# zadorlab/sella

Hardware: AMD Instinct MI355X
Metric: Davidson iterations/s (3N=3072 synthetic Hessian, jd0, gamma=0.1, maxiter=40; whole rayleigh_ritz call incl. device eigh of the preconditioner) (higher is better)
Workload: dtype f64; 1 GPU; 1024-atom-equivalent 3N=3072 fp64 Davidson (BASELINE configs[1]), one independent replica per GPU; n=3072, maxiter=40, method=jd0, problems=20, matrices=4

## Files before the change

### sella_amd/csrc/eigh.hip

```cpp
#include "internal.h"
#include "host_math.h"
#include "secular.h"

#include <algorithm>
#include <chrono>
#include <numeric>

namespace sella {
namespace {

constexpr int TRD_NBMAX = 64;
constexpr int TRD_PA = 1;
constexpr int WY_NB = 32;

__device__ __forceinline__ double wave_sum_e(double v) { return wave_sum64(v); }

__device__ __forceinline__ double block_sum_256(double v, double* red ) {
    v = wave_sum_e(v);
    __syncthreads();
    if ((threadIdx.x & 63) == 0) red[threadIdx.x >> 6] = v;
    __syncthreads();
    return red[0] + red[1] + red[2] + red[3];
}

struct TrdRowArgs {
    double* A; int ld, n;
    int j;
    int i;
    int do_row;
    double* Vp; double* Wp; int ldp;
    const double* u_prev; double* u_cur;
    const double* wraw;
    const double* partA_prev; int nblkA_prev;
    double* partA_cur;
    const double* partB; int nblkB;
    const double* colscal;
    const double* cdots;
    double* dvec;
};

template <int IPC>
__global__ __launch_bounds__(256) void trd_row_kernel(TrdRowArgs a) {
    __shared__ double red[4];
    SELLA_ARG(a.A); SELLA_ARG(a.ld); SELLA_ARG(a.n); SELLA_ARG(a.j); SELLA_ARG(a.i); SELLA_ARG(a.do_row); SELLA_ARG(a.Vp);
    SELLA_ARG(a.Wp); SELLA_ARG(a.ldp); SELLA_ARG(a.u_cur); SELLA_ARG(a.wraw); SELLA_ARG(a.partA_cur); SELLA_ARG(a.partB);
    SELLA_ARG(a.nblkB); SELLA_ARG(a.colscal); SELLA_ARG(a.cdots); SELLA_ARG(a.dvec);
    const int tid = threadIdx.x;
    const int j = a.j, i = a.i, ldp = a.ldp;
    const int c = j + blockIdx.x * 256 + tid;
    const bool valid = c < a.n;
    const int cl = valid ? c : a.n - 1;
    const int ip = i - 1;
    double pv0[8];
    {
        const int last = (a.nblkB > 0) ? a.nblkB - 1 : 0;
#pragma unroll
        for (int k = 0; k < 8; ++k) {
            const int b = tid + 256 * k;
            pv0[k] = a.partB[b < a.nblkB ? b : last];
        }
    }
    auto sum_partials = [&]() -> double {
        double vw = 0.0;
        if (IPC > 0 || i > 0) {
#pragma unroll
// ... 22 lines not shown
    bool vw_done = false;
    if (IPC > 3) {
        __shared__ double uni[4 * 32];
        constexpr int NPC = IPC > 0 ? IPC : 1;
        double vcs[NPC], wcs[NPC];
#pragma unroll
        for (int p = 0; p < NPC; ++p) {
            vcs[p] = a.Vp[(size_t)p * ldp + cl];
            wcs[p] = a.Wp[(size_t)p * ldp + cl];
        }
        if (tid < 4 * NPC) {
            const int p = tid >> 2, k = tid & 3;
            uni[tid] = (k == 0) ? a.cdots[p] : (k == 1) ? a.cdots[TRD_NBMAX + p]
                     : (k == 2) ? a.Vp[(size_t)p * ldp + j] : a.Wp[(size_t)p * ldp + j];
        }
        vw = block_sum_256(sum_partials(), red);
        vw_done = true;
#pragma unroll
        for (int p = 0; p < NPC; ++p) {
            const double c1 = uni[4 * p], c2 = uni[4 * p + 1], vj = uni[4 * p + 2], wj_p = uni[4 * p + 3];
            s += vcs[p] * c1 + wcs[p] * c2;
            q += vcs[p] * wj_p + wcs[p] * vj;
            cc += c1 * c2;
            t += vj * c1 + wj_p * c2;
        }
    } else {
#pragma unroll
        for (int p = 0; p < np; ++p) {
            const double c1 = a.cdots[p], c2 = a.cdots[TRD_NBMAX + p];
            const double vj = a.Vp[(size_t)p * ldp + j], wj_p = a.Wp[(size_t)p * ldp + j];
            const double vc = a.Vp[(size_t)p * ldp + cl], wcp = a.Wp[(size_t)p * ldp + cl];
            s += vc * c1 + wcp * c2;
            q += vc * wj_p + wcp * vj;
            cc += c1 * c2;
            t += vj * c1 + wj_p * c2;
        }
    }
    double wc = 0.0, u = 0.0;
    if (i > 0) {
        if (!vw_done) vw = block_sum_256(sum_partials(), red);
        const double alpha2 = -0.5 * tau * tau * (vw - 2.0 * cc);
        const double wj = tau * (wrawj - t) + alpha2;
        wc = tau * (wrawc - s) + alpha2 * vprev;
        if (valid) a.Wp[(size_t)ip * ldp + c] = wc;
        u = arow - q - (vprev * wj + wc);
    } else {
        u = arow;
    }
    if (!a.do_row) return;
    if (valid) {
        a.u_cur[c] = u;
        if (c == j) a.dvec[j] = u;
    }
    double ss = (valid && c >= j + 2) ? u * u : 0.0;
    ss = block_sum_256(ss, red);
    if (tid == 0) a.partA_cur[(size_t)blockIdx.x * TRD_PA] = ss;
}

__device__ __forceinline__ double2 ldg2(const double* p) { return *reinterpret_cast<const double2*>(p); }

struct TrdGemvArgs {
    const double* A22;
    int ld, m, shift, o, n, j;
    int pad;
    const double* ubuf;
    const double* partA; int nblkA;
    double* wraw;
    double* partB;
    double* Vrow;
    double* Arow;
    double* taus; double* evec; double* colscal;
    const double* Wp; const double* Vp; int ldp, i;
    double* cdots;
};

template <int NCH>
__global__ __launch_bounds__(256) void trd_gemv_kernel(TrdGemvArgs a) {
    __shared__ double red[4][2];
    const int lane = threadIdx.x & 63, wave = threadIdx.x >> 6;
    const int row0 = blockIdx.x * 2 - a.pad;
    const int mtot = a.m + 2 * a.i;
    const int oc = a.o - a.shift;
    const double2* arow[2];
    double lead[2];
#pragma unroll
    for (int r = 0; r < 2; ++r) {
        int rr = row0 + r;
        if (rr < 0) rr = 0;
        if (rr > mtot - 1) rr = mtot - 1;
        const double* base;
        if (rr < a.m) base = a.A22 + (size_t)rr * a.ld;
        else if (rr < a.m + a.i) base = a.Wp + (size_t)(rr - a.m) * a.ldp + oc;
        else base = a.Vp + (size_t)(rr - a.m - a.i) * a.ldp + oc;
        arow[r] = reinterpret_cast<const double2*>(base);
        lead[r] = base[a.shift];
    }
    double ssl0 = a.partA[(size_t)(lane < a.nblkA ? lane : a.nblkA - 1) * TRD_PA];
    double ssl = 0.0;
    for (int b = lane + 64; b < a.nblkA; b += 64) ssl += a.partA[(size_t)b * TRD_PA];
    const double alpha = a.ubuf[a.o];
    double urow[2];
#pragma unroll
    for (int r = 0; r < 2; ++r) {
        const int rr = row0 + r;
        urow[r] = a.ubuf[(rr >= 0 && rr < a.m) ? a.o + rr : a.o];
    }
    double acc[2] = {0.0, 0.0};
    const int n2 = (a.m + a.shift + 1) >> 1;
    auto uval = [&](int cabs) -> double { return (cabs > a.o && cabs < a.n) ? a.ubuf[cabs] : 0.0; };
// ... 1914 lines not shown
                hipLaunchKernelGGL(zhat_batched_kernel, dim3((maxK + 3) / 4, nm), dim3(256), 0, c->stream, mdd, Dd, wd, taud,
                                   orgd, zhd);
                hipLaunchKernelGGL(build_u_batched_kernel, dim3(maxK, nm), dim3(256), 0, c->stream, mdd, Dd, zhd, taud, orgd,
                                   W.Ut, ld);
            }
            hipLaunchKernelGGL(gather_level_kernel, dim3((maxN + 255) / 256, n), dim3(256), 0, c->stream, mdd, mrowd, idxd, cur,
                               W.Zc, nxt, ld);
            HIPCHK(hipGetLastError());
            SCHK(launch_gemm_merge_batched(c, nm, gdescd, maxN, maxK, W.Ut, W.Zc, nxt, ld));
        }
        HIPCHK(hipGetLastError());
        HIPCHK(hipMemcpyAsync(lam, lamd, (size_t)n * sizeof(double), hipMemcpyDeviceToHost, c->stream));
        HIPCHK(hipMemcpyAsync(hi2, info, 2 * sizeof(int), hipMemcpyDeviceToHost, c->stream));
        std::swap(cur, nxt);
        if (dc_timing) {
            const auto tw3 = std::chrono::steady_clock::now();
            auto us = [](auto a, auto b) { return std::chrono::duration<double, std::micro>(b - a).count(); };
            fprintf(stderr, "dc level %d: wait %.1f us, values + plan + staging %.1f us, uploads + launches %.1f us\n", h, us(tw0, tw1),
                    us(tw1, tw2), us(tw2, tw3));
        }
        if (pipelined) {
            plans_prev.swap(plans);
            if (h < maxdepth) SCHK(queue_level_vectors(h + 1, cur));
        } else {
            SCHK(stream_wait(c));
            SCHK(take_level_values(plans, defl_all[h & 1]));
        }
    }
    if (pipelined && maxdepth >= 1) {
        SCHK(stream_wait(c));
        SCHK(take_level_values(plans_prev, defl_all[maxdepth & 1]));
    }
    order.resize(n);
    ascending_order(vals.data(), n, order.data(), order_all.data());
    for (int i = 0; i < n; ++i) wout[i] = vals[order[i]];
    std::copy(order.begin(), order.end(), hidx);
    HIPCHK(hipMemcpyAsync(idxd, hidx, (size_t)n * sizeof(int), hipMemcpyHostToDevice, c->stream));
    SCHK(launch_gather_rows(c, cur, ld, idxd, n, n, nxt, ld));
    SCHK(stream_wait(c));
    if (nxt != W.Za) std::swap(W.Za, W.Zb);
    return SELLA_OK;
}

static int tridiagonalise(EighWork& W, double* taus, double* dvec, double* evec) {
    sella_ctx* c = W.c;
    const int n = W.n, ld = W.ld;
    int nb = (int)c->opt.eigh_nb;
    if (nb > TRD_NBMAX) nb = TRD_NBMAX;
    const int nrefl = n - 2;
    double *Vp, *Wp, *part;
    SCHK(scratch_get(c, SCR_MISC0, (size_t)2 * TRD_NBMAX * ld * sizeof(double), &Vp));
    Wp = Vp + (size_t)nb * ld;
    HIPCHK(s_memset0(c, Vp, (size_t)2 * nb * ld * sizeof(double)));
    const int maxblkA = (n + 255) / 256 + 1, maxblkB = (n + 16 + 2 * TRD_NBMAX + 1) / 2 + 1;
    SCHK(scratch_get(c, SCR_MISC1, ((size_t)2 * maxblkA * TRD_PA + 2 * (size_t)maxblkB + 4 * TRD_NBMAX + 128) * sizeof(double), &part));
    double* partA[2] = {part, part + (size_t)maxblkA * TRD_PA};
    double* partB = part + 2 * (size_t)maxblkA * TRD_PA;
    double* ub[2] = {W.vec + (size_t)V_U0 * ld, W.vec + (size_t)V_U1 * ld};
    double* wraw = W.vec + (size_t)V_WRAW * ld;
    double* colscal = W.vec + (size_t)V_COL * ld;
    double* cdots = partB + maxblkB + 8;
    double* partB2[2] = {partB, cdots + 2 * TRD_NBMAX + 8};
    double* colscal2[2] = {colscal, partB2[1] + maxblkB + 8};
    double* wraw2[2] = {wraw, W.vec + (size_t)V_WRAW2 * ld};
    const int upd_max = (int)c->opt.eigh_upd_max;
    int cur = 0, nblkA_prev = 0, nblkB_prev = 0;
    const int symv_min = (int)c->opt.eigh_symv_min;
    const int symTR = c->opt.eigh_symv_tr == 128 ? 128 : 64;
    const int symNJ = (n + SYMV_TC - 1) / SYMV_TC, symNI = (n + symTR - 1) / symTR;
    const int ldP = (n + 255) / 256 * 256;
    double *Prow = nullptr, *Pcol = nullptr;
    if (symv_min > 0 && n - 1 >= symv_min) {
        SCHK(scratch_get(c, SCR_SYMV, (size_t)(symNJ + symNI) * ldP * sizeof(double), &Prow));
        Pcol = Prow + (size_t)symNJ * ldP;
    }
    const int tail_lds = (int)std::min<long>(c->opt.eigh_tail_lds, TRD_TAIL);
    bool lower_stale = false;
    const bool can_tri = c->opt.rank2k_stream;
    for (int j0 = 0; j0 < nrefl; j0 += nb) {
        const int kb = std::min(nb, nrefl - j0);
        if (upd_max > 0 && !lower_stale && n - j0 - 1 <= upd_max && !(tail_lds > 0 && n - j0 <= tail_lds) &&
            !(symv_min > 0 && n - j0 - 1 >= symv_min)) {
            const int jend = tail_lds > 0 ? std::min(nrefl, n - tail_lds) : nrefl;
            int fc = 0, nblk_last = 0;
            for (int j = j0; j < jend; ++j) {
                const int o = j + 1, m = n - o;
                TrdUpdArgs ua;
                ua.A = W.A; ua.ld = ld; ua.n = n; ua.j = j;
                ua.o = o; ua.m = m; ua.oc = o & ~1; ua.shift = o - ua.oc;
                ua.v_prev = ub[1 - fc]; ua.v_cur = ub[fc];
                ua.wraw_prev = wraw2[1 - fc]; ua.wraw_cur = wraw2[fc];
                ua.partB_prev = partB2[1 - fc]; ua.nblkB_prev = nblk_last; ua.partB_cur = partB2[fc];
                ua.colscal_prev = colscal2[1 - fc]; ua.colscal_cur = colscal2[fc];
                ua.taus = taus; ua.evec = evec; ua.dvec = dvec;
                int R = (int)c->opt.eigh_upd_rows;
                if (R != 2 && R != 4 && R != 8) R = 2;
                while (R < 8 && (8 * R + m + R - 1) / R > TRD_UPD_MAXGRID) R *= 2;
                ua.pad = o % (8 * R);
                const int grid = (ua.pad + m + R - 1) / R;
                if (grid > TRD_UPD_MAXGRID) { set_error("eigh_upd_max too large for the one-launch-per-column chain"); return SELLA_E_INVALID; }
                const int n2 = (m + ua.shift + 1) >> 1;
                const int nt_max = (int)c->opt.eigh_upd_nt;
                const bool first = j == j0;
                const bool prof_all = c->prof;
                if (prof_all && (j & 3)) c->prof = false;
                if (c->prof) SCHK(stream_wait(c));
                prof_begin(c, PROF_OTHER, (first ? 8.0 : 16.0) * m * (double)m, (first ? 2.0 : 6.0) * m * (double)m);
#define SELLA_TRD_UPD(RR, NT)                                                                                             \
    do {                                                                                                                  \
        if (first) SELLA_LAUNCH(c, HIP_KERNEL_NAME(trd_upd_kernel<RR, NT, true>), dim3(grid), dim3(NT), 0, ua);           \
        else SELLA_LAUNCH(c, HIP_KERNEL_NAME(trd_upd_kernel<RR, NT, false>), dim3(grid), dim3(NT), 0, ua);                \
    } while (0)
#define SELLA_TRD_UPD_NT(RR)                                                                                              \
    do {                                                                                                                  \
        if (nt_max <= 128 || n2 <= 128) SELLA_TRD_UPD(RR, 128);                                                           \
        else if (nt_max <= 256 || n2 <= 256) SELLA_TRD_UPD(RR, 256);                                                      \
        else SELLA_TRD_UPD(RR, 512);                                                                                      \
    } while (0)
                switch (R) {
                    case 2: SELLA_TRD_UPD_NT(2); break;
                    case 4: SELLA_TRD_UPD_NT(4); break;
                    default: SELLA_TRD_UPD_NT(8); break;
                }
#undef SELLA_TRD_UPD_NT
#undef SELLA_TRD_UPD
                prof_end(c);
                c->prof = prof_all;
                nblk_last = grid;
                fc = 1 - fc;
            }
            if (jend > j0) {
                TrdUpdFinishArgs fa;
                fa.A = W.A; fa.ld = ld; fa.n = n; fa.o = jend;
                fa.v = ub[1 - fc]; fa.wraw = wraw2[1 - fc];
                fa.partB = partB2[1 - fc]; fa.nblkB = nblk_last;
                fa.colscal = colscal2[1 - fc];
                SELLA_LAUNCH(c, trd_upd_finish_kernel, dim3((n - jend + 3) / 4), dim3(256), 0, fa);
            }
            HIPCHK(hipGetLastError());
            j0 = jend - nb;
            continue;
        }
        if (tail_lds > 0 && n - j0 <= tail_lds) {
            prof_begin(c, PROF_OTHER, 8.0 * (n - j0) * (double)(n - j0), 0.0);
            SELLA_LAUNCH(c, trd_tail_lds_kernel, dim3(1), dim3(1024), 0, W.A, ld, n, j0, dvec, evec, taus);
            prof_end(c);
            HIPCHK(hipGetLastError());
            return SELLA_OK;
        }
        const bool panel_symv = symv_min > 0 && n - j0 - 1 >= symv_min;
        for (int i = 0; i <= kb; ++i) {
            const int j = j0 + i;
            const bool do_row = i < kb;
            TrdRowArgs ra;
            ra.A = W.A; ra.ld = ld; ra.n = n; ra.j = j; ra.i = i; ra.do_row = do_row ? 1 : 0;
            ra.Vp = Vp; ra.Wp = Wp; ra.ldp = ld;
            ra.u_prev = ub[1 - cur]; ra.u_cur = ub[cur];
            ra.wraw = wraw;
            ra.partA_prev = partA[1 - cur]; ra.nblkA_prev = nblkA_prev;
            ra.partA_cur = partA[cur];
            ra.partB = partB; ra.nblkB = nblkB_prev;
            ra.colscal = colscal;
            ra.cdots = cdots;
            ra.dvec = dvec;
            const int nblkA = (n - j + 255) / 256;
            const dim3 gA(nblkA), bA(256);
            const bool prof_all = c->prof;
            if (prof_all && (j & 3)) c->prof = false;
            if (c->prof) SCHK(stream_wait(c));
            prof_begin(c, PROF_OTHER, 8.0 * (2.0 * i + 3.0) * (n - j), 0.0);
            switch (i - 1) {
#define SELLA_TRD_ROW_CASE(IP) case IP: SELLA_LAUNCH(c, HIP_KERNEL_NAME(trd_row_kernel<IP>), gA, bA, 0, ra); break;
                case -1:
                SELLA_TRD_ROW_CASE(0) SELLA_TRD_ROW_CASE(1) SELLA_TRD_ROW_CASE(2) SELLA_TRD_ROW_CASE(3)
                SELLA_TRD_ROW_CASE(4) SELLA_TRD_ROW_CASE(5) SELLA_TRD_ROW_CASE(6) SELLA_TRD_ROW_CASE(7)
                SELLA_TRD_ROW_CASE(8) SELLA_TRD_ROW_CASE(9) SELLA_TRD_ROW_CASE(10) SELLA_TRD_ROW_CASE(11)
                SELLA_TRD_ROW_CASE(12) SELLA_TRD_ROW_CASE(13) SELLA_TRD_ROW_CASE(14) SELLA_TRD_ROW_CASE(15)
                SELLA_TRD_ROW_CASE(16) SELLA_TRD_ROW_CASE(17) SELLA_TRD_ROW_CASE(18) SELLA_TRD_ROW_CASE(19)
                SELLA_TRD_ROW_CASE(20) SELLA_TRD_ROW_CASE(21) SELLA_TRD_ROW_CASE(22) SELLA_TRD_ROW_CASE(23)
                SELLA_TRD_ROW_CASE(24) SELLA_TRD_ROW_CASE(25) SELLA_TRD_ROW_CASE(26) SELLA_TRD_ROW_CASE(27)
                SELLA_TRD_ROW_CASE(28) SELLA_TRD_ROW_CASE(29) SELLA_TRD_ROW_CASE(30) SELLA_TRD_ROW_CASE(31)
#undef SELLA_TRD_ROW_CASE
                default: SELLA_LAUNCH(c, HIP_KERNEL_NAME(trd_row_kernel<-1>), gA, bA, 0, ra);
            }
            prof_end(c);
            if (!do_row) { c->prof = prof_all; break; }
            const int o = j + 1, m = n - o, oc = o & ~1;
            TrdGemvArgs ga;
            ga.A22 = W.A + (size_t)o * ld + oc; ga.ld = ld; ga.m = m; ga.shift = o - oc; ga.o = o; ga.n = n; ga.j = j;
            ga.ubuf = ub[cur];
            ga.partA = partA[cur]; ga.nblkA = nblkA;
            ga.wraw = wraw; ga.partB = partB;
            ga.Vrow = Vp + (size_t)i * ld;
            ga.Arow = W.A + (size_t)j * ld;
            ga.taus = taus; ga.evec = evec; ga.colscal = colscal;
            ga.Wp = Wp; ga.Vp = Vp; ga.ldp = ld; ga.i = i; ga.cdots = cdots;
            ga.pad = o - (o / 16) * 16;
            int nblkB = (ga.pad + m + 2 * i + 1) / 2;
            if (panel_symv) {
                TrdSymvArgs sa;
                sa.A = W.A; sa.ld = ld; sa.n = n; sa.o = o; sa.ubuf = ub[cur];
                sa.Prow = Prow; sa.Pcol = Pcol; sa.ldp = ldP;
                prof_begin(c, PROF_TRD_GEMV, 4.0 * m * (double)m, 2.0 * m * (double)m);
                if (symTR == 128) SELLA_LAUNCH(c, trd_symv_kernel<128>, dim3(symNJ, symNI), dim3(256), 0, sa);
                else SELLA_LAUNCH(c, trd_symv_kernel<64>, dim3(symNJ, symNI), dim3(256), 0, sa);
                prof_end(c);
                TrdSymvFinishArgs fa;
                fa.A = W.A; fa.ld = ld; fa.n = n; fa.o = o; fa.j = j; fa.ubuf = ub[cur];
                fa.partA = partA[cur]; fa.nblkA = nblkA;
                fa.Prow = Prow; fa.Pcol = Pcol; fa.ldp = ldP;
                fa.wraw = wraw; fa.partB = partB; fa.Vrow = ga.Vrow; fa.Arow = ga.Arow;
                fa.taus = taus; fa.evec = evec; fa.colscal = colscal;
                fa.Wp = Wp; fa.Vp = Vp; fa.ldpan = ld; fa.i = i; fa.cdots = cdots;
                fa.tr = symTR;
                fa.nelem = (n - (o & ~63) + 63) / 64;
                nblkB = fa.nelem;
                prof_begin(c, PROF_OTHER, 16.0 * m * (double)(m / symTR + m / SYMV_TC), 0.0);
                SELLA_LAUNCH(c, trd_symv_finish_kernel, dim3(fa.nelem + 2 * i), dim3(256), 0, fa);
                prof_end(c);
            } else {
                prof_begin(c, PROF_TRD_GEMV, 8.0 * m * (double)m, 2.0 * m * (double)m);
                const int n2g = (m + ga.shift + 1) >> 1;
                const int nch = c->opt.eigh_gemv_flat ? (n2g + 255) / 256 : 1 << 30;
                if (nch <= 2) SELLA_LAUNCH(c, trd_gemv_kernel<2>, dim3(nblkB), dim3(256), 0, ga);
                else if (nch <= 4) SELLA_LAUNCH(c, trd_gemv_kernel<4>, dim3(nblkB), dim3(256), 0, ga);
                else if (nch <= 6) SELLA_LAUNCH(c, trd_gemv_kernel<6>, dim3(nblkB), dim3(256), 0, ga);
                else if (nch <= 8) SELLA_LAUNCH(c, trd_gemv_kernel<8>, dim3(nblkB), dim3(256), 0, ga);
                else if (nch <= 10) SELLA_LAUNCH(c, trd_gemv_kernel<10>, dim3(nblkB), dim3(256), 0, ga);
                else SELLA_LAUNCH(c, trd_gemv_kernel<0>, dim3(nblkB), dim3(256), 0, ga);
                prof_end(c);
            }
            c->prof = prof_all;
            nblkA_prev = nblkA;
            nblkB_prev = nblkB;
            cur = 1 - cur;
        }
        HIPCHK(hipGetLastError());
        const int r0 = j0 + kb, mt = n - r0;
        if (mt > 0) {
            double* At = W.A + (size_t)r0 * ld + r0;
            const bool next_symv = symv_min > 0 && n - r0 - 1 >= symv_min;
            const bool aligned = !(ld & 1) && !(reinterpret_cast<uintptr_t>(At) & 15);
            if (lower_stale && !(can_tri && aligned)) {
                SCHK(launch_mirror_upper(c, At, mt, ld));
                lower_stale = false;
            }
            if (can_tri && aligned && (next_symv || lower_stale)) {
                SCHK(launch_rank2k_stream(c, At, mt, ld, Vp + r0, Wp + r0, ld, kb, -1.0, true));
                lower_stale = true;
                if (!next_symv) {
                    SCHK(launch_mirror_upper(c, At, mt, ld));
                    lower_stale = false;
                }
            } else if (c->opt.rank2k_stream) SCHK(launch_rank2k_stream(c, At, mt, ld, Vp + r0, Wp + r0, ld, kb, -1.0));
            else SCHK(launch_sym_rank2k(c, At, mt, ld, Vp + r0, Wp + r0, ld, kb, -1.0));
        }
    }
    hipLaunchKernelGGL(tridiag_tail_kernel, dim3(1), dim3(64), 0, c->stream, W.A, ld, n, dvec, evec, taus);
    HIPCHK(hipGetLastError());
    return SELLA_OK;
}

static int eig_rank1_update(sella_ctx* c, EighWork& W, int nr, int n, int ld, double* w, double* Vt, const double* q,
                            double sigma, const double* append_lam0 = nullptr, int* nr_out = nullptr) {
    double* zdev = W.vec + (size_t)V_Z * ld;
    double* csd = W.vec + (size_t)V_CS0 * ld;
    double* Dd = W.vec + (size_t)V_DD * ld;
    double* wd = W.vec + (size_t)V_WD * ld;
    double* taud = W.vec + (size_t)V_TAU * ld;
    double* zhd = W.vec + (size_t)V_ZH * ld;
    double* lamd = W.vec + (size_t)V_LAM * ld;
    int* info = W.ibuf;
    int* i1d = W.ibuf + 16;
    int* i2d = i1d + n;
    int* idxd = i1d + 2 * n;
    int* orgd = i1d + 3 * n;
    static const bool dbg_time = getenv("SELLA_DEBUG_TIMING") != nullptr;
    auto now = [] { return std::chrono::duration<double>(std::chrono::steady_clock::now().time_since_epoch()).count(); };
    const double tt0 = now();
    const int nr_in = nr;
    if (append_lam0) {
        double* slot = Vt + (size_t)nr * ld;
        HIPCHK(s_memcpy(c, slot, q, (size_t)ld * sizeof(double), hipMemcpyDeviceToDevice));
        SCHK(gs_project_twice(c, Vt, ld, nr, slot, n));
        ++nr;
    }
    SCHK(launch_gemv_rows(c, Vt, nr, n, ld, q, ld, 1, zdev, ld, GemvEpi()));
    void* stage;
    SCHK(host_stage(c, (4 * (size_t)ld + 2 * (size_t)n + 8) * sizeof(double) + (3 * (size_t)n + 16) * sizeof(int), &stage));
    double* hcs = static_cast<double*>(stage);
    double* hD = hcs + 2 * (size_t)ld;
    double* hw = hcs + 3 * (size_t)ld;
    double* z = hcs + 4 * (size_t)ld;
    double* lam = z + n;
    int* hinfo = reinterpret_cast<int*>(lam + n + 8);
    int* hr1 = hinfo + 8;
    int* hr2 = hr1 + n;
    int* hidx = hr1 + 2 * (size_t)n;
    HIPCHK(hipMemcpyAsync(z, zdev, (size_t)nr * sizeof(double), hipMemcpyDeviceToHost, c->stream));
    HIPCHK(s_memset0(c, info, 8 * sizeof(int)));
    if (append_lam0) SCHK(sync_scalars(c, 8, 3));
    else SCHK(stream_wait(c));
    if (append_lam0) {
        const double n0sq = c->hscal[8], n1 = sqrt(c->hscal[9]), n2 = sqrt(c->hscal[10]);
        bool kept = (n0sq > 0.0) && (n1 == n1) && !(n1 < 1e-13) && (n2 == n2) && !(n2 < 1e-13);
        if (kept && fabs(1.0 - n2) > 1e-15) {
// ... 668 lines not shown
```

### sella_amd/csrc/internal.h

```cpp
#pragma once
#include <hip/hip_runtime.h>
#include <hip/hip_ext.h>

#include <stdarg.h>
#include <stdio.h>
#include <string.h>

#include <deque>
#include <map>
#include <string>
#include <vector>

#include "../../include/sella_hip.h"

#define SELLA_HD __host__ __device__
#include "small_linalg.h"
#include "cohort.h"

#if defined(__HIP_DEVICE_COMPILE__) && !defined(SELLA_NO_ARG_BATCH)
#define SELLA_PIN(x) asm volatile("" : "+v"(x))
#define SELLA_ARG(x) asm volatile("" : : "s"(x))
#elif defined(__HIP_DEVICE_COMPILE__)
#define SELLA_PIN(x) asm volatile("" : "+v"(x))
#define SELLA_ARG(x) ((void)0)
// ... 190 lines not shown
    } while (0)

enum ScratchSlot {
    SCR_X = 0, SCR_Y, SCR_PART, SCR_V, SCR_AV, SCR_V2, SCR_AV2, SCR_R, SCR_T, SCR_W, SCR_C,
    SCR_EIG0, SCR_EIG1, SCR_EIG2, SCR_EIG3, SCR_EIG4, SCR_EIG5, SCR_EIG6, SCR_UPD0, SCR_UPD1, SCR_UPD2,
    SCR_UPD3, SCR_UPD4, SCR_QR0, SCR_QR1, SCR_STEP0, SCR_STEP1, SCR_STEP2, SCR_MISC0, SCR_MISC1, SCR_PSMALL, SCR_SYMV, SCR_NSLOTS
};

struct GemvEpi {
    int mode = 0;
    const double* dvec = nullptr;
    double theta = 0, alpha = 1, beta = 0;
};
struct GemvX {
    const double* p[8];
};
int launch_gemv_rows(sella_ctx* c, const double* A, int rows, int cols, int lda, const double* X,
                     int ldx, int nrhs, double* Y, int ldy, const GemvEpi& epi);
int launch_gemv_rows_xp(sella_ctx* c, const double* A, int rows, int cols, int lda,
                        const double* const* xs, int nrhs, double* Y, int ldy, const GemvEpi& epi);
int launch_gemv_rows2(sella_ctx* c, const double* A, int rows, int lda, const double* A2, int rows2, int lda2, int cols,
                      const double* x, double* y, double* y2);
int launch_panel16(sella_ctx* c, const double* A, int rows, int cols, int lda, const double* Xp, int nrhs,
                   double* Y, int ldy);
int launch_panel16_marked(sella_ctx* c, const double* A, int rows, int cols, int lda, const double* Xp, int nrhs, double* Y,
                          int ldy);
int launch_normalize(sella_ctx* c, double* x, int n, double* out);
int launch_gemv_cols(sella_ctx* c, const double* A, int rows, int cols, int lda, const double* X,
                     int ldx, int nrhs, double* Y, int ldy);
int launch_lincomb(sella_ctx* c, int n, int nout, const double* P1, int ldp1, int k1,
                   const double* W1, int ldw1, const double* P2, int ldp2, int k2,
                   const double* W2, int ldw2, double beta, double* out, int ldo);
int launch_rows_sumsq(sella_ctx* c, const double* P, int ldp, int nrows, int n, double* out);
int launch_scale_by(sella_ctx* c, double* x, int n, const double* scal, int mode);
int launch_jd_combine(sella_ctx* c, const double* x, const double* y, const double* dots,
                      double* t, int n);
int launch_axpby(sella_ctx* c, int n, double a, const double* x, double b, const double* y,
                 double* z);
int launch_axpby2d(sella_ctx* c, int rows, int cols, double a, const double* A, int lda, double b,
                   const double* B, int ldb, double* C, int ldc);
int launch_transpose(sella_ctx* c, const double* A, int rows, int cols, int lda, double* At,
                     int ldat);
int launch_gemm(sella_ctx* c, int transA, int transB, int M, int N, int K, double alpha,
                const double* A, int lda, const double* B, int ldb, double beta, double* C,
                int ldc);
int launch_symmetrize(sella_ctx* c, double* B, int n, int ld);
int gs_orthonormalise(sella_ctx* c, const double* basis, int ldb, int k, double* t, int n,
                      double eps1, double eps2, int maxiter, int* kept, double* first_norm);
int gs_project_twice(sella_ctx* c, const double* basis, int ldb, int k, double* t, int n);
int launch_sym_rank2k(sella_ctx* c, double* B, int n, int ld, const double* Up, const double* Zp,
                      int ldp, int kk, double alpha = 1.0);
int launch_rank2k_stream(sella_ctx* c, double* C, int m, int ld, const double* Up, const double* Zp, int ldp, int kk,
                         double alpha, bool upper_only = false);
int launch_mirror_upper(sella_ctx* c, double* C, int m, int ld);
int eig_lowrank_update(sella_ctx* c, int n, double* w, Mat* V, Mat* Vt, const double* Up, const double* Zp,
                       int ldp, int kk, int* nrank1);
int lr_lowrank_update(sella_ctx* c, int n, int* r_io, double* mu, double lam0, Mat* Wt, const double* Up, const double* Zp,
                      int ldp, int kk, int* nrank1);
int internals_queue(sella_ctx* c, int natoms, int nc, const double* dpos, const double* dtv, double* dq, double* dgrad,
                    double* dhess);
int sparse_int_ncoords(const sella_sparse_int* s);
int sparse_int_natoms(const sella_sparse_int* s);
int emt_eval_resident(sella_ctx* c, int n, const double* pos, const double* par, int nshift, const double* shifts,
                      const double* dconst, double rc, double acut, double cutoff, double beta, double* energy, double* grad,
                      double* virial6 = nullptr);
int emt_queue(sella_ctx* c, int n, const double* pos, const double* par, int nshift, const double* shifts, const double* dconst,
              double rc, double acut, double cutoff, double beta, double** eatom, double** grad, bool virial = false);
int emt_hessian_resident(sella_ctx* c, int n, const double* pos, const double* par, int nshift, const double* shifts,
                         const double* dconst, double rc, double acut, double cutoff, double beta, sella_mat out);
int emt_hvp_resident(sella_ctx* c, int n, const double* pos, const double* par, int nshift, const double* shifts,
                     const double* dconst, double rc, double acut, double cutoff, double beta, const double* V, int k, double* HV);
int calc_queue(sella_calc* k, const double* x, double** g_dev, double** aux_dev, int* naux);
double calc_finish(sella_calc* k, const double* x, const double* aux_host);
int hvp_device_apply(sella_hvp* op, const double* x, double* y);
int hvp_device_apply_block(sella_hvp* op, const double* X, int ldx, int nh, double* Y, int ldy);
long hvp_calls(const sella_hvp* op);
int hvp_dim(const sella_hvp* op);
sella_ctx* hvp_ctx(const sella_hvp* op);
int stepper_from_panel(sella_ctx* c, int kind, const double* src, int ld, const int* idx, int m, int n, const double* ev,
                       const double* gh, int order, sella_stepper** out);
int stepper_on_panel(sella_ctx* c, int kind, const double* src, int ld, const int* idx, int m, int n, const double* ev,
                     const double* gh, int order, sella_stepper** out);
void stepper_panel_scale(sella_stepper* st, int mode, double factor);
void stepper_set_fast_search(sella_stepper* st, bool on, bool boundary_hint = false);
void stepper_set_alpha_hint(sella_stepper* st, double hint);
double stepper_alpha_found(const sella_stepper* st);
struct CalcPipe {
    sella_calc* calc = nullptr;
    const double* x = nullptr;
    double* g_out = nullptr;
    double f = 0.0;
    bool done = false;
};
int lr_fused_step(sella_ctx* c, sella_opt_step_t* a, bool* handled, CalcPipe* pipe = nullptr);
int opt_step_with_calc(sella_ctx* c, sella_opt_step_t* a, sella_calc* calc, const double* x, double* g_new, double* f_new,
                       bool* force_call_made = nullptr);
int launch_gemm_merge_batched(sella_ctx* c, int nbatch, const int* desc, int maxN, int maxK, const double* A,
                              const double* B, double* C, int ld);
int launch_gather_rows(sella_ctx* c, const double* in, int ldi, const int* idx, int nrows,
                       int ncols, double* out, int ldo);

}
```

### sella_amd/csrc/update.hip

```cpp
#include "internal.h"
#include <chrono>
#include <cstdlib>
#include <cstdint>
#include "host_math.h"

namespace sella {

constexpr int R2K_KT = 16;

__device__ __forceinline__ void sym_rank2k_vb(const VB vb, double* __restrict__ B, int n, int ld,
                                                         const double* __restrict__ Up,
                                                         const double* __restrict__ Zp, int ldp, int kk,
                                                         double alpha) {
    if (vb.x < vb.y) return;
    __shared__ double t1[32][33];
    __shared__ double t2[32][33];
    __shared__ double ur[R2K_KT][32], zr[R2K_KT][32], uc[R2K_KT][32], zc[R2K_KT][32];
    const int tx = threadIdx.x & 31, ty = threadIdx.x >> 5;
    const int r0 = vb.y * 32, c0 = vb.x * 32;
    for (int k = ty; k < 32; k += 8) {
        int r = r0 + k, cc = c0 + tx;
        t1[k][tx] = (r < n && cc < n) ? B[(size_t)r * ld + cc] : 0.0;
        r = c0 + k; cc = r0 + tx;
        t2[k][tx] = (r < n && cc < n) ? B[(size_t)r * ld + cc] : 0.0;
    }
    double acc[4] = {0.0, 0.0, 0.0, 0.0};
    for (int a0 = 0; a0 < kk; a0 += R2K_KT) {
        const int at = (kk - a0 < R2K_KT) ? (kk - a0) : R2K_KT;
        __syncthreads();
        for (int t = threadIdx.x; t < R2K_KT * 32; t += 256) {
            const int a = t >> 5, i = t & 31;
            const bool ok = a < at;
            const int gr = r0 + i, gc = c0 + i;
            ur[a][i] = (ok && gr < n) ? Up[(size_t)(a0 + a) * ldp + gr] : 0.0;
            zr[a][i] = (ok && gr < n) ? Zp[(size_t)(a0 + a) * ldp + gr] : 0.0;
            uc[a][i] = (ok && gc < n) ? Up[(size_t)(a0 + a) * ldp + gc] : 0.0;
            zc[a][i] = (ok && gc < n) ? Zp[(size_t)(a0 + a) * ldp + gc] : 0.0;
        }
        __syncthreads();
#pragma unroll
        for (int a = 0; a < R2K_KT; ++a) {
            const double ucx = uc[a][tx], zcx = zc[a][tx];
#pragma unroll
            for (int q = 0; q < 4; ++q) acc[q] += ur[a][ty + 8 * q] * zcx + zr[a][ty + 8 * q] * ucx;
        }
    }
    __syncthreads();
#pragma unroll
    for (int q = 0; q < 4; ++q) {
        const int k = ty + 8 * q;
        const double v = 0.5 * (t1[k][tx] + t2[tx][k]) + alpha * acc[q];
        t1[k][tx] = v;
    }
    __syncthreads();
    const bool diag = (vb.x == vb.y);
    for (int k = ty; k < 32; k += 8) {
        int r = r0 + k, cc = c0 + tx;
        const double v = (diag && k > tx) ? t1[tx][k] : t1[k][tx];
        if (r < n && cc < n) B[(size_t)r * ld + cc] = v;
        if (!diag) {
            r = c0 + k; cc = r0 + tx;
            if (r < n && cc < n) B[(size_t)r * ld + cc] = t1[tx][k];
        }
    }
}
__global__ __launch_bounds__(256) void sym_rank2k_kernel(double* __restrict__ B, int n, int ld,
                                                         const double* __restrict__ Up,
                                                         const double* __restrict__ Zp, int ldp, int kk,
                                                         double alpha) { sym_rank2k_vb(vb_hw(), B, n, ld, Up, Zp, ldp, kk, alpha); }

typedef double upd_f64x4 __attribute__((ext_vector_type(4)));
constexpr int RS_TR = 32, RS_TC = 128;

__global__ __launch_bounds__(256) void rank2k_stream_kernel(double* __restrict__ C, int m, int ld,
                                                            const double* __restrict__ Up,
                                                            const double* __restrict__ Zp, int ldp, int kk,
                                                            double alpha) {
    __shared__ double dl[RS_TR][RS_TC + 2];
    const int tid = threadIdx.x, lane = tid & 63, wave = tid >> 6;
    const int li = lane & 15, lq = lane >> 4;
    const int r0 = blockIdx.y * RS_TR, c0 = blockIdx.x * RS_TC;
    const int wr = r0 + 16 * (wave & 1);
    const int wc = c0 + 64 * (wave >> 1);
    upd_f64x4 acc[4];
#pragma unroll
    for (int t = 0; t < 4; ++t) acc[t] = upd_f64x4{0.0, 0.0, 0.0, 0.0};
    const int rr = (wr + li < m) ? wr + li : m - 1;
    const int K = 2 * kk;
    for (int k0 = 0; k0 < K; k0 += 4) {
        const int k = k0 + lq;
        const bool ok = k < K;
        const int kc = ok ? k : 0;
        const double* xrow = (kc < kk) ? Up + (size_t)kc * ldp : Zp + (size_t)(kc - kk) * ldp;
        const double* yrow = (kc < kk) ? Zp + (size_t)kc * ldp : Up + (size_t)(kc - kk) * ldp;
        const double a = ok ? xrow[rr] : 0.0;
#pragma unroll
        for (int t = 0; t < 4; ++t) {
            const int cc = wc + 16 * t + li;
            const double b = (ok && cc < m) ? yrow[cc] : 0.0;
            acc[t] = __builtin_amdgcn_mfma_f64_16x16x4f64(a, b, acc[t], 0, 0, 0);
        }
    }
#pragma unroll
    for (int t = 0; t < 4; ++t)
#pragma unroll
        for (int q = 0; q < 4; ++q) dl[16 * (wave & 1) + lq + 4 * q][64 * (wave >> 1) + 16 * t + li] = acc[t][q];
    __syncthreads();
    const int pc = tid & 63, pr = tid >> 6;
#pragma unroll
    for (int s8 = 0; s8 < RS_TR; s8 += 4) {
        const int r = r0 + s8 + pr, cidx = c0 + 2 * pc;
        if (r < m && cidx < m) {
            double* p = C + (size_t)r * ld + cidx;
            const double d0 = dl[s8 + pr][2 * pc], d1 = dl[s8 + pr][2 * pc + 1];
            if (cidx + 1 < m) {
                double2 v = *reinterpret_cast<double2*>(p);
                v.x += alpha * d0;
                v.y += alpha * d1;
                *reinterpret_cast<double2*>(p) = v;
            } else {
                p[0] += alpha * d0;
            }
        }
    }
}

template <int KK>
__global__ __launch_bounds__(256) void rank2k_stream_fixed_kernel(double* __restrict__ C, int m, int ld,
                                                                  const double* __restrict__ Up,
                                                                  const double* __restrict__ Zp, int ldp, double alpha,
                                                                  int upper_only) {
    __shared__ double dl[RS_TR][RS_TC + 2];
    constexpr int KS = 2 * KK / 4;
    if (upper_only && (int)(blockIdx.x * RS_TC + RS_TC - 1) < (int)(blockIdx.y * RS_TR)) return;
    const int tid = threadIdx.x, lane = tid & 63, wave = tid >> 6;
    const int li = lane & 15, lq = lane >> 4;
    const int r0 = blockIdx.y * RS_TR, c0 = blockIdx.x * RS_TC;
    const int wr = r0 + 16 * (wave & 1);
    const int wc = c0 + 64 * (wave >> 1);
    const int rr = (wr + li < m) ? wr + li : m - 1;
    double av[KS], bv[KS][4];
#pragma unroll
    for (int s = 0; s < KS; ++s) {
        const int k = 4 * s + lq;
        const double* xrow = (k < KK) ? Up + (size_t)k * ldp : Zp + (size_t)(k - KK) * ldp;
        const double* yrow = (k < KK) ? Zp + (size_t)k * ldp : Up + (size_t)(k - KK) * ldp;
        av[s] = xrow[rr];
#pragma unroll
        for (int t = 0; t < 4; ++t) {
            const int cc = wc + 16 * t + li;
            bv[s][t] = yrow[cc < m ? cc : m - 1];
        }
    }
    const int pc = tid & 63, pr = tid >> 6;
    const int cidx = c0 + 2 * pc;
    double2 cv[RS_TR / 4];
    {
        const int cl = (cidx < m) ? cidx : 0;
#pragma unroll
        for (int q = 0; q < RS_TR / 4; ++q) {
            const int r = (r0 + 4 * q + pr < m) ? r0 + 4 * q + pr : m - 1;
            cv[q] = *reinterpret_cast<const double2*>(C + (size_t)r * ld + cl);
        }
    }
#pragma unroll
    for (int s = 0; s < KS; ++s)
#pragma unroll
        for (int t = 0; t < 4; ++t) bv[s][t] = (wc + 16 * t + li < m) ? bv[s][t] : 0.0;
    upd_f64x4 acc[4];
#pragma unroll
    for (int t = 0; t < 4; ++t) acc[t] = upd_f64x4{0.0, 0.0, 0.0, 0.0};
#pragma unroll
    for (int s = 0; s < KS; ++s)
#pragma unroll
        for (int t = 0; t < 4; ++t) acc[t] = __builtin_amdgcn_mfma_f64_16x16x4f64(av[s], bv[s][t], acc[t], 0, 0, 0);
#pragma unroll
    for (int t = 0; t < 4; ++t)
#pragma unroll
        for (int q = 0; q < 4; ++q) dl[16 * (wave & 1) + lq + 4 * q][64 * (wave >> 1) + 16 * t + li] = acc[t][q];
    __syncthreads();
#pragma unroll
    for (int q = 0; q < RS_TR / 4; ++q) {
        const int r = r0 + 4 * q + pr;
        if (r < m && cidx < m) {
            double* p = C + (size_t)r * ld + cidx;
            const double d0 = dl[4 * q + pr][2 * pc], d1 = dl[4 * q + pr][2 * pc + 1];
            if (cidx + 1 < m) {
                double2 v = cv[q];
                v.x += alpha * d0;
                v.y += alpha * d1;
                *reinterpret_cast<double2*>(p) = v;
            } else {
                p[0] = cv[q].x + alpha * d0;
            }
        }
    }
}

__device__ __forceinline__ void mirror_upper_vb(const VB vb, double* __restrict__ C, int m, int ld) {
    __shared__ double t[32][33];
    const int bi = vb.y, bj = vb.x;
    if (bj < bi) return;
    const int tx = threadIdx.x & 31, ty = threadIdx.x >> 5;
    for (int q = 0; q < 4; ++q) {
        const int r = bi * 32 + ty + 8 * q, cc = bj * 32 + tx;
        t[ty + 8 * q][tx] = (r < m && cc < m) ? C[(size_t)r * ld + cc] : 0.0;
    }
    __syncthreads();
    for (int q = 0; q < 4; ++q) {
        const int r = bj * 32 + ty + 8 * q, cc = bi * 32 + tx;
        if (r < m && cc < m && r > cc) C[(size_t)r * ld + cc] = t[tx][ty + 8 * q];
    }
}
__global__ __launch_bounds__(256) void mirror_upper_kernel(double* __restrict__ C, int m, int ld) { mirror_upper_vb(vb_hw(), C, m, ld); }

int launch_mirror_upper(sella_ctx* c, double* C, int m, int ld) {
    if (m <= 1) return SELLA_OK;
    const int nt = (m + 31) / 32;
    prof_begin(c, PROF_OTHER, 8.0 * m * (double)m, 0.0);
    SELLA_LAUNCHB_PROF(c, mirror_upper_kernel, mirror_upper_vb, 256, dim3(nt, nt), dim3(256), 0, C, m, ld);
    prof_end(c);
    HIPCHK(hipGetLastError());
    return SELLA_OK;
}

int launch_rank2k_stream(sella_ctx* c, double* C, int m, int ld, const double* Up, const double* Zp, int ldp, int kk,
                         double alpha, bool upper_only) {
    if (m <= 0 || kk <= 0) return SELLA_OK;
    if ((ld & 1) || (reinterpret_cast<uintptr_t>(C) & 15)) return launch_sym_rank2k(c, C, m, ld, Up, Zp, ldp, kk, alpha);
    const double part = upper_only ? 0.5 : 1.0;
    prof_begin(c, PROF_UPDATE, part * 16.0 * m * (double)m, part * 4.0 * kk * (double)m * m);
    const dim3 grid((m + RS_TC - 1) / RS_TC, (m + RS_TR - 1) / RS_TR);
    const int uo = upper_only ? 1 : 0;
    if (kk == 16 && c->opt.rank2k_fixed)
        SELLA_LAUNCH(c, rank2k_stream_fixed_kernel<16>, grid, dim3(256), 0, C, m, ld, Up, Zp, ldp, alpha, uo);
    else if (kk == 32 && c->opt.rank2k_fixed)
        SELLA_LAUNCH(c, rank2k_stream_fixed_kernel<32>, grid, dim3(256), 0, C, m, ld, Up, Zp, ldp, alpha, uo);
    else
    SELLA_LAUNCH(c, rank2k_stream_kernel, grid, dim3(256), 0, C, m, ld, Up,
                 Zp, ldp, kk, alpha);
    prof_end(c);
    HIPCHK(hipGetLastError());
    return SELLA_OK;
}

int launch_sym_rank2k(sella_ctx* c, double* B, int n, int ld, const double* Up, const double* Zp, int ldp,
                      int kk, double alpha) {
    prof_begin(c, PROF_UPDATE, 16.0 * n * (double)n, 4.0 * kk * (double)n * n);
    const int nb = (n + 31) / 32;
    SELLA_LAUNCHB_PROF(c, sym_rank2k_kernel, sym_rank2k_vb, 256, dim3(nb, nb), dim3(256), 0, B, n, ld, Up, Zp, ldp, kk, alpha);
    prof_end(c);
    HIPCHK(hipGetLastError());
    return SELLA_OK;
}

namespace {

using hostm::vec;

int gram(sella_ctx* c, const double* P, int ka, const double* Q, int kb, int n, int ld, vec& G) {
    G.assign((size_t)ka * kb, 0.0);
    if (ka * kb > DS_STAGE - DS_CVEC) { set_error("update: too many secant pairs"); return SELLA_E_UNSUPPORTED; }
    double* d = c->dscal + DS_CVEC;
    SCHK(launch_gemv_rows(c, P, ka, n, ld, Q, ld, kb, d, ka, GemvEpi()));
    SCHK(read_scalars(c, DS_CVEC, ka * kb));
    for (int a = 0; a < ka; ++a)
        for (int b = 0; b < kb; ++b) G[(size_t)a * kb + b] = c->hscal[DS_CVEC + (size_t)b * ka + a];
    return SELLA_OK;
}

int put_k(sella_ctx* c, const vec& h, size_t offset, double** d) {
    double* base;
    SCHK(scratch_get(c, SCR_W, (size_t)(1 << 16) * sizeof(double), &base));
    if (offset + h.size() > (size_t)(1 << 16)) { set_error("update: coefficient buffer overflow"); return SELLA_E_UNSUPPORTED; }
    SCHK(h2d_async(c, base + offset, h.data(), h.size() * sizeof(double)));
    *d = base + offset;
    return SELLA_OK;
}

int symmetrize_panels(sella_ctx* c, const double* Sp, const double* Yp, int n, int k, int ld, int symm,
                      double* Ytp) {
    SCHK(launch_axpby2d(c, k, n, 1.0, Yp, ld, 0.0, nullptr, 0, Ytp, ld));
    if (symm < 0 || k == 1) return SELLA_OK;
    if (symm > 2) { set_error("Unknown symmetrization method %d", symm); return SELLA_E_INVALID; }
    vec STS, STY, X((size_t)k * k);
    SCHK(gram(c, Sp, k, Sp, k, n, ld, STS));
    SCHK(gram(c, Sp, k, Yp, k, n, ld, STY));
    const int which = hostm::symm_coeffs(k, STS.data(), STY.data(), symm, X.data());
    if (which < 0) return SELLA_OK;
    double* dX;
    SCHK(put_k(c, X, 0, &dX));
    return launch_lincomb(c, n, k, which == 0 ? Sp : Yp, ld, k, dX, k, nullptr, 0, 0, nullptr, 0, 1.0, Ytp, ld);
}

bool invert(int k, const vec& M, vec& Minv) {
    vec LU(M);
// ... 464 lines not shown
```

Before: 537.5 davidson_iter/s.

## Fuse first row of next panel into rank-2k trailing update kernel

The rank-2k stream kernel that updates the trailing matrix now also writes the first updated row as the next panel's u vector, stores its diagonal, and emits per-wave sum-of-squares partials. This lets the next panel skip its i==0 trd_row_kernel launch, removing one launch and one serial dependency per panel. The row kernel's norm reduction also switches from a block-wide sum with two syncthreads to per-wave partials, with the partial buffer enlarged to match. In exchange there is extra seam bookkeeping, a fixed-kernel path where row 0 may be skipped by the upper_only early return (upper_only is 0 here), and wider argument structs.

```diff
diff --git a/sella_amd/csrc/eigh.hip b/sella_amd/csrc/eigh.hip
--- a/sella_amd/csrc/eigh.hip
+++ b/sella_amd/csrc/eigh.hip
@@ -11,6 +11,7 @@
 
 constexpr int TRD_NBMAX = 64;
 constexpr int TRD_PA = 1;
+constexpr int TRD_PAW = 4;
 constexpr int WY_NB = 32;
 
 __device__ __forceinline__ double wave_sum_e(double v) { return wave_sum64(v); }
@@ -139,9 +140,8 @@
         a.u_cur[c] = u;
         if (c == j) a.dvec[j] = u;
     }
-    double ss = (valid && c >= j + 2) ? u * u : 0.0;
-    ss = block_sum_256(ss, red);
-    if (tid == 0) a.partA_cur[(size_t)blockIdx.x * TRD_PA] = ss;
+    const double ss = wave_sum_e((valid && c >= j + 2) ? u * u : 0.0);
+    if ((tid & 63) == 0) a.partA_cur[(size_t)(TRD_PAW * blockIdx.x + (tid >> 6)) * TRD_PA] = ss;
 }
 
 __device__ __forceinline__ double2 ldg2(const double* p) { return *reinterpret_cast<const double2*>(p); }
@@ -2162,7 +2162,7 @@
     SCHK(scratch_get(c, SCR_MISC0, (size_t)2 * TRD_NBMAX * ld * sizeof(double), &Vp));
     Wp = Vp + (size_t)nb * ld;
     HIPCHK(s_memset0(c, Vp, (size_t)2 * nb * ld * sizeof(double)));
-    const int maxblkA = (n + 255) / 256 + 1, maxblkB = (n + 16 + 2 * TRD_NBMAX + 1) / 2 + 1;
+    const int maxblkA = TRD_PAW * ((n + 255) / 256) + 1, maxblkB = (n + 16 + 2 * TRD_NBMAX + 1) / 2 + 1;
     SCHK(scratch_get(c, SCR_MISC1, ((size_t)2 * maxblkA * TRD_PA + 2 * (size_t)maxblkB + 4 * TRD_NBMAX + 128) * sizeof(double), &part));
     double* partA[2] = {part, part + (size_t)maxblkA * TRD_PA};
     double* partB = part + 2 * (size_t)maxblkA * TRD_PA;
@@ -2187,10 +2187,14 @@
     const int tail_lds = (int)std::min<long>(c->opt.eigh_tail_lds, TRD_TAIL);
     bool lower_stale = false;
     const bool can_tri = c->opt.rank2k_stream;
+    auto to_lds_tail = [&](int jn) { return tail_lds > 0 && n - jn <= tail_lds; };
+    auto to_upd_chain = [&](int jn) {
+        return upd_max > 0 && n - jn - 1 <= upd_max && !to_lds_tail(jn) && !(symv_min > 0 && n - jn - 1 >= symv_min);
+    };
+    bool seam_done = false;
     for (int j0 = 0; j0 < nrefl; j0 += nb) {
         const int kb = std::min(nb, nrefl - j0);
-        if (upd_max > 0 && !lower_stale && n - j0 - 1 <= upd_max && !(tail_lds > 0 && n - j0 <= tail_lds) &&
-            !(symv_min > 0 && n - j0 - 1 >= symv_min)) {
+        if (!lower_stale && to_upd_chain(j0)) {
             const int jend = tail_lds > 0 ? std::min(nrefl, n - tail_lds) : nrefl;
             int fc = 0, nblk_last = 0;
             for (int j = j0; j < jend; ++j) {
@@ -2251,7 +2255,7 @@
             j0 = jend - nb;
             continue;
         }
-        if (tail_lds > 0 && n - j0 <= tail_lds) {
+        if (to_lds_tail(j0)) {
             prof_begin(c, PROF_OTHER, 8.0 * (n - j0) * (double)(n - j0), 0.0);
             SELLA_LAUNCH(c, trd_tail_lds_kernel, dim3(1), dim3(1024), 0, W.A, ld, n, j0, dvec, evec, taus);
             prof_end(c);
@@ -2273,27 +2277,31 @@
             ra.colscal = colscal;
             ra.cdots = cdots;
             ra.dvec = dvec;
-            const int nblkA = (n - j + 255) / 256;
-            const dim3 gA(nblkA), bA(256);
+            const bool seam_row = i == 0 && seam_done;
+            const dim3 gA((n - j + 255) / 256), bA(256);
+            const int nblkA = seam_row ? nblkA_prev : TRD_PAW * (int)gA.x;
             const bool prof_all = c->prof;
             if (prof_all && (j & 3)) c->prof = false;
             if (c->prof) SCHK(stream_wait(c));
-            prof_begin(c, PROF_OTHER, 8.0 * (2.0 * i + 3.0) * (n - j), 0.0);
-            switch (i - 1) {
+            if (!seam_row) {
+                prof_begin(c, PROF_OTHER, 8.0 * (2.0 * i + 3.0) * (n - j), 0.0);
+                switch (i - 1) {
 #define SELLA_TRD_ROW_CASE(IP) case IP: SELLA_LAUNCH(c, HIP_KERNEL_NAME(trd_row_kernel<IP>), gA, bA, 0, ra); break;
-                case -1:
-                SELLA_TRD_ROW_CASE(0) SELLA_TRD_ROW_CASE(1) SELLA_TRD_ROW_CASE(2) SELLA_TRD_ROW_CASE(3)
-                SELLA_TRD_ROW_CASE(4) SELLA_TRD_ROW_CASE(5) SELLA_TRD_ROW_CASE(6) SELLA_TRD_ROW_CASE(7)
-                SELLA_TRD_ROW_CASE(8) SELLA_TRD_ROW_CASE(9) SELLA_TRD_ROW_CASE(10) SELLA_TRD_ROW_CASE(11)
-                SELLA_TRD_ROW_CASE(12) SELLA_TRD_ROW_CASE(13) SELLA_TRD_ROW_CASE(14) SELLA_TRD_ROW_CASE(15)
-                SELLA_TRD_ROW_CASE(16) SELLA_TRD_ROW_CASE(17) SELLA_TRD_ROW_CASE(18) SELLA_TRD_ROW_CASE(19)
-                SELLA_TRD_ROW_CASE(20) SELLA_TRD_ROW_CASE(21) SELLA_TRD_ROW_CASE(22) SELLA_TRD_ROW_CASE(23)
-                SELLA_TRD_ROW_CASE(24) SELLA_TRD_ROW_CASE(25) SELLA_TRD_ROW_CASE(26) SELLA_TRD_ROW_CASE(27)
-                SELLA_TRD_ROW_CASE(28) SELLA_TRD_ROW_CASE(29) SELLA_TRD_ROW_CASE(30) SELLA_TRD_ROW_CASE(31)
+                    case -1:
+                    SELLA_TRD_ROW_CASE(0) SELLA_TRD_ROW_CASE(1) SELLA_TRD_ROW_CASE(2) SELLA_TRD_ROW_CASE(3)
+                    SELLA_TRD_ROW_CASE(4) SELLA_TRD_ROW_CASE(5) SELLA_TRD_ROW_CASE(6) SELLA_TRD_ROW_CASE(7)
+                    SELLA_TRD_ROW_CASE(8) SELLA_TRD_ROW_CASE(9) SELLA_TRD_ROW_CASE(10) SELLA_TRD_ROW_CASE(11)
+                    SELLA_TRD_ROW_CASE(12) SELLA_TRD_ROW_CASE(13) SELLA_TRD_ROW_CASE(14) SELLA_TRD_ROW_CASE(15)
+                    SELLA_TRD_ROW_CASE(16) SELLA_TRD_ROW_CASE(17) SELLA_TRD_ROW_CASE(18) SELLA_TRD_ROW_CASE(19)
+                    SELLA_TRD_ROW_CASE(20) SELLA_TRD_ROW_CASE(21) SELLA_TRD_ROW_CASE(22) SELLA_TRD_ROW_CASE(23)
+                    SELLA_TRD_ROW_CASE(24) SELLA_TRD_ROW_CASE(25) SELLA_TRD_ROW_CASE(26) SELLA_TRD_ROW_CASE(27)
+                    SELLA_TRD_ROW_CASE(28) SELLA_TRD_ROW_CASE(29) SELLA_TRD_ROW_CASE(30) SELLA_TRD_ROW_CASE(31)
 #undef SELLA_TRD_ROW_CASE
-                default: SELLA_LAUNCH(c, HIP_KERNEL_NAME(trd_row_kernel<-1>), gA, bA, 0, ra);
-            }
-            prof_end(c);
+                    default: SELLA_LAUNCH(c, HIP_KERNEL_NAME(trd_row_kernel<-1>), gA, bA, 0, ra);
+                }
+                prof_end(c);
+            }
+            seam_done = false;
             if (!do_row) { c->prof = prof_all; break; }
             const int o = j + 1, m = n - o, oc = o & ~1;
             TrdGemvArgs ga;
@@ -2362,6 +2370,10 @@
                     SCHK(launch_mirror_upper(c, At, mt, ld));
                     lower_stale = false;
                 }
+            } else if (c->opt.rank2k_stream && aligned && r0 < nrefl && !to_upd_chain(r0) && !to_lds_tail(r0)) {
+                const Rank2kSeam seam = {ub[cur] + r0, dvec + r0, partA[cur]};
+                SCHK(launch_rank2k_stream_seam(c, At, mt, ld, Vp + r0, Wp + r0, ld, kb, -1.0, seam, &nblkA_prev));
+                seam_done = true;
             } else if (c->opt.rank2k_stream) SCHK(launch_rank2k_stream(c, At, mt, ld, Vp + r0, Wp + r0, ld, kb, -1.0));
             else SCHK(launch_sym_rank2k(c, At, mt, ld, Vp + r0, Wp + r0, ld, kb, -1.0));
         }
diff --git a/sella_amd/csrc/internal.h b/sella_amd/csrc/internal.h
--- a/sella_amd/csrc/internal.h
+++ b/sella_amd/csrc/internal.h
@@ -266,6 +266,9 @@
                       int ldp, int kk, double alpha = 1.0);
 int launch_rank2k_stream(sella_ctx* c, double* C, int m, int ld, const double* Up, const double* Zp, int ldp, int kk,
                          double alpha, bool upper_only = false);
+struct Rank2kSeam { double* u; double* d; double* partA; };
+int launch_rank2k_stream_seam(sella_ctx* c, double* C, int m, int ld, const double* Up, const double* Zp, int ldp, int kk,
+                              double alpha, const Rank2kSeam& seam, int* npart);
 int launch_mirror_upper(sella_ctx* c, double* C, int m, int ld);
 int eig_lowrank_update(sella_ctx* c, int n, double* w, Mat* V, Mat* Vt, const double* Up, const double* Zp,
                        int ldp, int kk, int* nrank1);
diff --git a/sella_amd/csrc/update.hip b/sella_amd/csrc/update.hip
--- a/sella_amd/csrc/update.hip
+++ b/sella_amd/csrc/update.hip
@@ -72,10 +72,31 @@
 typedef double upd_f64x4 __attribute__((ext_vector_type(4)));
 constexpr int RS_TR = 32, RS_TC = 128;
 
-__global__ __launch_bounds__(256) void rank2k_stream_kernel(double* __restrict__ C, int m, int ld,
-                                                            const double* __restrict__ Up,
-                                                            const double* __restrict__ Zp, int ldp, int kk,
-                                                            double alpha) {
+struct Rank2kStreamArgs {
+    double* C; int m, ld;
+    const double* Up; const double* Zp; int ldp, kk;
+    double alpha;
+    int upper_only;
+    double* seam_u; double* seam_d; double* seam_partA;
+};
+
+__device__ __forceinline__ void rank2k_seam_row(const Rank2kStreamArgs& a, int cidx, double ux, double uy) {
+    const bool ok0 = cidx < a.m, ok1 = cidx + 1 < a.m;
+    if (ok0) a.seam_u[cidx] = ux;
+    if (ok1) a.seam_u[cidx + 1] = uy;
+    if (cidx == 0) a.seam_d[0] = ux;
+    double s = (ok0 && cidx >= 2) ? ux * ux : 0.0;
+    s = (ok1 && cidx >= 2) ? fma(uy, uy, s) : s;
+    s = wave_sum64(s);
+    if ((threadIdx.x & 63) == 0) a.seam_partA[blockIdx.x] = s;
+}
+
+__global__ __launch_bounds__(256) void rank2k_stream_kernel(Rank2kStreamArgs a) {
+    double* __restrict__ C = a.C;
+    const double* __restrict__ Up = a.Up;
+    const double* __restrict__ Zp = a.Zp;
+    const int m = a.m, ld = a.ld, ldp = a.ldp, kk = a.kk;
+    const double alpha = a.alpha;
     __shared__ double dl[RS_TR][RS_TC + 2];
     const int tid = threadIdx.x, lane = tid & 63, wave = tid >> 6;
     const int li = lane & 15, lq = lane >> 4;
@@ -93,12 +114,12 @@
         const int kc = ok ? k : 0;
         const double* xrow = (kc < kk) ? Up + (size_t)kc * ldp : Zp + (size_t)(kc - kk) * ldp;
         const double* yrow = (kc < kk) ? Zp + (size_t)kc * ldp : Up + (size_t)(kc - kk) * ldp;
-        const double a = ok ? xrow[rr] : 0.0;
+        const double xa = ok ? xrow[rr] : 0.0;
 #pragma unroll
         for (int t = 0; t < 4; ++t) {
             const int cc = wc + 16 * t + li;
-            const double b = (ok && cc < m) ? yrow[cc] : 0.0;
-            acc[t] = __builtin_amdgcn_mfma_f64_16x16x4f64(a, b, acc[t], 0, 0, 0);
+            const double yb = (ok && cc < m) ? yrow[cc] : 0.0;
+            acc[t] = __builtin_amdgcn_mfma_f64_16x16x4f64(xa, yb, acc[t], 0, 0, 0);
         }
     }
 #pragma unroll
@@ -110,26 +131,31 @@
 #pragma unroll
     for (int s8 = 0; s8 < RS_TR; s8 += 4) {
         const int r = r0 + s8 + pr, cidx = c0 + 2 * pc;
+        double2 v = make_double2(0.0, 0.0);
         if (r < m && cidx < m) {
             double* p = C + (size_t)r * ld + cidx;
             const double d0 = dl[s8 + pr][2 * pc], d1 = dl[s8 + pr][2 * pc + 1];
             if (cidx + 1 < m) {
-                double2 v = *reinterpret_cast<double2*>(p);
+                v = *reinterpret_cast<double2*>(p);
                 v.x += alpha * d0;
                 v.y += alpha * d1;
                 *reinterpret_cast<double2*>(p) = v;
             } else {
-                p[0] += alpha * d0;
+                v.x = p[0] + alpha * d0;
+                p[0] = v.x;
             }
         }
+        if (s8 == 0 && a.seam_u && r == 0) rank2k_seam_row(a, cidx, v.x, v.y);
     }
 }
 
 template <int KK>
-__global__ __launch_bounds__(256) void rank2k_stream_fixed_kernel(double* __restrict__ C, int m, int ld,
-                                                                  const double* __restrict__ Up,
-                                                                  const double* __restrict__ Zp, int ldp, double alpha,
-                                                                  int upper_only) {
+__global__ __launch_bounds__(256) void rank2k_stream_fixed_kernel(Rank2kStreamArgs a) {
+    double* __restrict__ C = a.C;
+    const double* __restrict__ Up = a.Up;
+    const double* __restrict__ Zp = a.Zp;
+    const int m = a.m, ld = a.ld, ldp = a.ldp, upper_only = a.upper_only;
+    const double alpha = a.alpha;
     __shared__ double dl[RS_TR][RS_TC + 2];
     constexpr int KS = 2 * KK / 4;
     if (upper_only && (int)(blockIdx.x * RS_TC + RS_TC - 1) < (int)(blockIdx.y * RS_TR)) return;
@@ -182,18 +208,20 @@
 #pragma unroll
     for (int q = 0; q < RS_TR / 4; ++q) {
         const int r = r0 + 4 * q + pr;
+        double2 v = cv[q];
         if (r < m && cidx < m) {
             double* p = C + (size_t)r * ld + cidx;
             const double d0 = dl[4 * q + pr][2 * pc], d1 = dl[4 * q + pr][2 * pc + 1];
             if (cidx + 1 < m) {
-                double2 v = cv[q];
                 v.x += alpha * d0;
                 v.y += alpha * d1;
                 *reinterpret_cast<double2*>(p) = v;
             } else {
-                p[0] = cv[q].x + alpha * d0;
+                v.x += alpha * d0;
+                p[0] = v.x;
             }
         }
+        if (q == 0 && a.seam_u && r == 0) rank2k_seam_row(a, cidx, v.x, v.y);
     }
 }
 
@@ -224,24 +252,36 @@
     return SELLA_OK;
 }
 
+static int rank2k_stream_launch(sella_ctx* c, const Rank2kStreamArgs& a) {
+    const int m = a.m, kk = a.kk;
+    const double part = a.upper_only ? 0.5 : 1.0;
+    prof_begin(c, PROF_UPDATE, part * 16.0 * m * (double)m, part * 4.0 * kk * (double)m * m);
+    const dim3 grid((m + RS_TC - 1) / RS_TC, (m + RS_TR - 1) / RS_TR);
+    if (kk == 16 && c->opt.rank2k_fixed) SELLA_LAUNCH(c, rank2k_stream_fixed_kernel<16>, grid, dim3(256), 0, a);
+    else if (kk == 32 && c->opt.rank2k_fixed) SELLA_LAUNCH(c, rank2k_stream_fixed_kernel<32>, grid, dim3(256), 0, a);
+    else SELLA_LAUNCH(c, rank2k_stream_kernel, grid, dim3(256), 0, a);
+    prof_end(c);
+    HIPCHK(hipGetLastError());
+    return SELLA_OK;
+}
+
 int launch_rank2k_stream(sella_ctx* c, double* C, int m, int ld, const double* Up, const double* Zp, int ldp, int kk,
                          double alpha, bool upper_only) {
     if (m <= 0 || kk <= 0) return SELLA_OK;
     if ((ld & 1) || (reinterpret_cast<uintptr_t>(C) & 15)) return launch_sym_rank2k(c, C, m, ld, Up, Zp, ldp, kk, alpha);
-    const double part = upper_only ? 0.5 : 1.0;
-    prof_begin(c, PROF_UPDATE, part * 16.0 * m * (double)m, part * 4.0 * kk * (double)m * m);
-    const dim3 grid((m + RS_TC - 1) / RS_TC, (m + RS_TR - 1) / RS_TR);
-    const int uo = upper_only ? 1 : 0;
-    if (kk == 16 && c->opt.rank2k_fixed)
-        SELLA_LAUNCH(c, rank2k_stream_fixed_kernel<16>, grid, dim3(256), 0, C, m, ld, Up, Zp, ldp, alpha, uo);
-    else if (kk == 32 && c->opt.rank2k_fixed)
-        SELLA_LAUNCH(c, rank2k_stream_fixed_kernel<32>, grid, dim3(256), 0, C, m, ld, Up, Zp, ldp, alpha, uo);
-    else
-    SELLA_LAUNCH(c, rank2k_stream_kernel, grid, dim3(256), 0, C, m, ld, Up,
-                 Zp, ldp, kk, alpha);
-    prof_end(c);
-    HIPCHK(hipGetLastError());
-    return SELLA_OK;
+    const Rank2kStreamArgs a = {C, m, ld, Up, Zp, ldp, kk, alpha, upper_only ? 1 : 0, nullptr, nullptr, nullptr};
+    return rank2k_stream_launch(c, a);
+}
+
+int launch_rank2k_stream_seam(sella_ctx* c, double* C, int m, int ld, const double* Up, const double* Zp, int ldp, int kk,
+                              double alpha, const Rank2kSeam& seam, int* npart) {
+    if (m <= 0 || kk <= 0 || (ld & 1) || (reinterpret_cast<uintptr_t>(C) & 15) || !seam.u || !seam.d || !seam.partA) {
+        set_error("rank2k_stream_seam: needs a non-empty 16-byte aligned block and all seam outputs");
+        return SELLA_E_INVALID;
+    }
+    const Rank2kStreamArgs a = {C, m, ld, Up, Zp, ldp, kk, alpha, 0, seam.u, seam.d, seam.partA};
+    *npart = (m + RS_TC - 1) / RS_TC;
+    return rank2k_stream_launch(c, a);
 }
 
 int launch_sym_rank2k(sella_ctx* c, double* B, int n, int ld, const double* Up, const double* Zp, int ldp,
```

Result: faster. 585.0 davidson_iter/s (median of 6 runs) (+8.8%).
